# tsurumeso/vocal-remover

Measured on NVIDIA H100. Metric: seconds-of-audio/sec separated (n_fft=2048, hop=1024), higher is better.
Workload: dtype bf16x3 (split-bf16 operands hi+lo, 3 wgmma passes, fp32 accumulate); fft/lstm fp32

## Files before the change

### vocal-remover_b200/build.py

```python
import os
import subprocess
import sys
from concurrent.futures import ThreadPoolExecutor

HERE = os.path.dirname(os.path.abspath(__file__))
CSRC = os.path.join(HERE, 'csrc')
OBJ = os.path.join(HERE, 'build')
LIB = os.path.join(HERE, 'libvr_b200.so')
SOURCES = ['api.cu', 'engine.cu', 'conv_simt.cu', 'conv_tc.cu', 'conv_tc_rows.cu', 'conv_tc_halo.cu', 'elementwise.cu', 'lstm.cu', 'fft.cu', 'resample.cu', 'flac.cu', 'flac_encode.cu']
NVCC = os.environ.get('NVCC', '/usr/local/cuda/bin/nvcc')
FLAGS = ['-gencode', 'arch=compute_90a,code=sm_90a', '-O3', '-lineinfo', '-std=c++17',
         '-Xcompiler', '-fPIC', '-Xcompiler', '-fvisibility=hidden', '--expt-relaxed-constexpr']


def _newest_header():
    hs = [os.path.join(CSRC, f) for f in os.listdir(CSRC) if f.endswith(('.h', '.cuh'))]
    hs.append(os.path.join(HERE, '..', 'include', 'vr_b200.h'))
    return max(os.path.getmtime(h) for h in hs)


def build(verbose=False, force=False):
    global OBJ, LIB
    extra = os.environ.get('VR_BUILD_FLAGS', '').split()
    if os.environ.get('VR_BUILD_TAG'):
        OBJ = os.path.join(HERE, 'build_' + os.environ['VR_BUILD_TAG'])
        LIB = os.path.join(HERE, 'libvr_b200_%s.so' % os.environ['VR_BUILD_TAG'])
    os.makedirs(OBJ, exist_ok=True)
    hdr = _newest_header()
    jobs = []
    for src in SOURCES:
        s = os.path.join(CSRC, src)
        o = os.path.join(OBJ, src.replace('.cu', '.o'))
        if force or not os.path.exists(o) or os.path.getmtime(o) < max(os.path.getmtime(s), hdr):
            jobs.append((s, o))

    def cc(job):
        s, o = job
        cmd = [NVCC] + FLAGS + extra + ['-c', s, '-o', o]
        if verbose:
            cmd += ['-Xptxas', '-v']
        r = subprocess.run(cmd, capture_output=True, text=True)
        if r.returncode != 0:
            raise RuntimeError('nvcc failed for %s:\n%s\n%s' % (s, r.stdout, r.stderr))
        return r.stderr

    with ThreadPoolExecutor(max_workers=min(8, max(1, len(jobs)))) as ex:
        logs = list(ex.map(cc, jobs))
    if verbose:
        for lg in logs:
            print(lg)
    objs = [os.path.join(OBJ, s.replace('.cu', '.o')) for s in SOURCES]
    if jobs or not os.path.exists(LIB):
        cmd = [NVCC, '-shared', '-o', LIB] + objs + ['-gencode', 'arch=compute_90a,code=sm_90a']
        r = subprocess.run(cmd, capture_output=True, text=True)
        if r.returncode != 0:
            raise RuntimeError('link failed:\n%s\n%s' % (r.stdout, r.stderr))
    return LIB


if __name__ == '__main__':
    print(build(verbose='-v' in sys.argv, force='-f' in sys.argv))
```

### vocal-remover_b200/csrc/api.cu

```cuda
#include <stdio.h>
#include <string.h>

#include <string>

#include "../../include/vr_b200.h"
#include "engine.h"
#include "kernels.h"
#include "tc_plan.h"

struct vr_ctx {
  vr::Engine* eng;
  std::string err;
};

static std::string g_create_err;

static int fail(vr_ctx* c, const std::string& m) {
  if (c) c->err = m;
  return -1;
}
static int done(vr_ctx* c, bool ok) {
  if (ok) return 0;
  c->err = c->eng->err;
  return -1;
// ... 255 lines not shown
  cudaError_t e = cudaMalloc(&p, (size_t)bytes);
  if (e != cudaSuccess) return fail(ctx, std::string("vr_shared_alloc: cudaMalloc: ") + cudaGetErrorString(e));
  cudaIpcMemHandle_t h;
  e = cudaIpcGetMemHandle(&h, p);
  if (e != cudaSuccess) {
    cudaFree(p);
    return fail(ctx, std::string("vr_shared_alloc: cudaIpcGetMemHandle: ") + cudaGetErrorString(e));
  }
  memcpy(handle64, &h, 64);
  *dev_ptr = p;
  return 0;
}

int vr_shared_open(vr_ctx* ctx, const unsigned char* handle64, void** dev_ptr) {
  CHECK_CTX(ctx);
  if (!dev_ptr || !handle64) return fail(ctx, "vr_shared_open: bad arguments");
  cudaIpcMemHandle_t h;
  memcpy(&h, handle64, 64);
  void* p = nullptr;
  cudaError_t e = cudaIpcOpenMemHandle(&p, h, cudaIpcMemLazyEnablePeerAccess);
  if (e != cudaSuccess) return fail(ctx, std::string("vr_shared_open: cudaIpcOpenMemHandle: ") + cudaGetErrorString(e));
  *dev_ptr = p;
  return 0;
}

int vr_shared_close(vr_ctx* ctx, void* dev_ptr, int32_t owner) {
  CHECK_CTX(ctx);
  if (!dev_ptr) return 0;
  cudaError_t e = owner ? cudaFree(dev_ptr) : cudaIpcCloseMemHandle(dev_ptr);
  if (e != cudaSuccess) return fail(ctx, std::string("vr_shared_close: ") + cudaGetErrorString(e));
  return 0;
}

int64_t vr_launch_count(const vr_ctx* ctx) { return ctx && ctx->eng ? ctx->eng->launches : 0; }

int vr_profile_enable(vr_ctx* ctx, int32_t on) {
  CHECK_CTX(ctx);
  ctx->eng->profile_enable(on != 0);
  return 0;
}

int vr_profile_read(vr_ctx* ctx, double* out6) {
  CHECK_CTX(ctx);
  return done(ctx, ctx->eng->profile_read(out6));
}

int vr_profile_dump(vr_ctx* ctx, char* text, int64_t cap, int64_t* needed) {
  CHECK_CTX(ctx);
  std::string t;
  if (!ctx->eng->profile_dump(t)) return done(ctx, false);
  if (needed) *needed = (int64_t)t.size() + 1;
  if (text && cap > 0) {
    const size_t n = t.size() < (size_t)cap - 1 ? t.size() : (size_t)cap - 1;
    memcpy(text, t.data(), n);
    text[n] = 0;
  }
  return 0;
}

int vr_debug_conv(vr_ctx* ctx, const float* x, int32_t N, int32_t Cin, int32_t H, int32_t W, const float* w,
                  const float* bias, int32_t Cout, int32_t k, int32_t stride, int32_t dil_h, int32_t dil_w, int32_t act,
                  int32_t use_tc, float* y, void* stream) {
  CHECK_CTX(ctx);
  return done(ctx, ctx->eng->debug_conv(x, N, Cin, H, W, w, bias, Cout, k, stride, dil_h, dil_w, act, use_tc, y,
                                        (cudaStream_t)stream));
}

int vr_debug_decoder(vr_ctx* ctx, const float* low, int32_t N, int32_t Cl, int32_t h, int32_t w, const float* skip,
                     int32_t Cs, const float* wgt, const float* bias, int32_t Cout, int32_t act, int32_t fused, float* y,
                     void* stream) {
  CHECK_CTX(ctx);
  return done(ctx, ctx->eng->debug_decoder(low, N, Cl, h, w, skip, Cs, wgt, bias, Cout, act, fused, y,
                                           (cudaStream_t)stream));
}

int vr_debug_tensor(vr_ctx* ctx, const char* name, int32_t n0, int32_t n, float* out, int64_t* shape4, void* stream) {
  CHECK_NET(ctx);
  if (!name || !shape4) return fail(ctx, "vr_debug_tensor: name and shape4 are required");
  return done(ctx, ctx->eng->debug_tensor(name, n0, n, out, shape4, (cudaStream_t)stream));
}

int vr_debug_set(int32_t key, int32_t value) {
  int* knob = key == 0 ? &vr::g_debug.trace : key == 2 ? &vr::g_debug.rows_wide : key == 3 ? &vr::g_debug.halo
            : key == 6 ? &vr::g_debug.kskip : key == 7 ? &vr::g_debug.crop_mask : nullptr;
  if (!knob) return -1;
  *knob = value;
  return 0;
}

int64_t vr_debug_trace(uint64_t* host_out, int64_t capacity) {
  return vr::tc_rows_read_trace((unsigned long long*)host_out, (long long)capacity);
}

}
```

### vocal-remover_b200/csrc/conv_tc.cu

```cuda
#include <cuda.h>
#include <stdio.h>

#include <map>
#include <tuple>

#include "engine.h"
#include "tc_common.cuh"
#include "tc_plan.h"

namespace vr {

static constexpr int kMaxStages = 8;
static constexpr int kConsumerWarps = 8;
static constexpr int kThreads = 32 * kConsumerWarps + 32;
static constexpr int kStaticSmem = 2048;

struct TcParams {
  int N, Ho, Wo, Wt, Ht, Nt, tiles_w, tiles_h, m_tiles, n_tiles;
  int stride, pad_h, pad_w, dil_h, dil_w, KW;
  int cchunks, total_sub, CinPadTC, Cout, act, stages;
  bf16* out_hi;
  bf16* out_lo;
  int64_t osn, osh;
  int osw;
// ... 73 lines not shown
    __syncwarp();
  } else {
    const int wg = warp >> 2;
    const float slope = act_slope(p.act);
    const uint32_t dhi = desc_hi(8 * KB * 2, kLayout);
    MbarRing ring(smem_u32(&bar_full[0]), smem_u32(&bar_empty[0]), 0, p.stages);
    float acc[BN / 2];
    for (int tile = blockIdx.x; tile < total_tiles; tile += gridDim.x) {
#pragma unroll
      for (int i = 0; i < BN / 2; ++i) acc[i] = 0.f;
      HeldSlot held;
      for (int it = 0; it < num_iters; ++it) {
        const int nsub = min(SUBS, p.total_sub - it * SUBS);
        ring.wait_full();
        const uint32_t sdesc = desc_lo(smem_base + (uint32_t)ring.slot * kStageBytes);
        wg_fence();
#pragma unroll
        for (int j = 0; j < SUBS; ++j) {
          if (j < nsub) {
            const uint32_t a_hi = sdesc + ((j * kASub + (uint32_t)wg * (kAPlane / 2)) >> 4);
            const uint32_t a_lo = a_hi + (kAPlane >> 4);
            const uint32_t b_hi = sdesc + ((kBRegion + j * kBSub) >> 4);
            const uint32_t b_lo = b_hi + (kBPlane >> 4);
#pragma unroll
            for (int k = 0; k < kSteps; ++k)
              wgmma_split3<BN>(acc, a_hi + 2u * k, a_lo + 2u * k, b_hi + 2u * k, b_lo + 2u * k, dhi);
          }
        }
        wg_commit();
        wg_wait<1>();
        held.release(ring, lane);
        held.hold(ring);
        ring.advance();
      }
      wg_wait<0>();
      held.release_last(ring, lane);

      const int nt = tile % p.n_tiles;
      const int mt = tile / p.n_tiles;
      const int w0 = (mt % p.tiles_w) * p.Wt;
      const int h0 = ((mt / p.tiles_w) % p.tiles_h) * p.Ht;
      const int n0 = (mt / (p.tiles_w * p.tiles_h)) * p.Nt;
      const int c_lane = nt * BN + 2 * (lane & 3);
#pragma unroll
      for (int hr = 0; hr < 2; ++hr) {
        const int row = 64 * wg + 16 * (warp & 3) + (lane >> 2) + 8 * hr;
        const int dw = row % p.Wt;
        const int dh = (row / p.Wt) % p.Ht;
        const int n = n0 + row / (p.Wt * p.Ht);
        if (n >= p.N) continue;
        const int64_t obase = (int64_t)n * p.osn + (int64_t)(h0 + dh) * p.osh + (int64_t)(w0 + dw) * p.osw;
#pragma unroll
        for (int j = 0; j < BN / 8; ++j)
          epilogue_pair(acc[4 * j + 2 * hr], acc[4 * j + 2 * hr + 1], bias_s, c_lane + 8 * j, p.Cout, slope,
                        p.out_hi + obase, p.out_lo + obase);
      }
    }
  }
}

#define VR_TC_FOR_BN(X, KB) X(KB, 16) X(KB, 32) X(KB, 48) X(KB, 64) X(KB, 80) X(KB, 96) X(KB, 112) X(KB, 128)
#define VR_TC_FOR_ALL(X) VR_TC_FOR_BN(X, 64) VR_TC_FOR_BN(X, 32) VR_TC_FOR_BN(X, 16)


TcDebug g_debug;

static constexpr int kMaxDevices = 64;
const TcDevice& tc_device() {
  static TcDevice table[kMaxDevices];
  static TcDevice none;
  int dev = -1;
  if (cudaGetDevice(&dev) != cudaSuccess || dev < 0 || dev >= kMaxDevices) return none;
  TcDevice& d = table[dev];
  if (!d.ok) {
    if (cudaDeviceGetAttribute(&d.max_smem, cudaDevAttrMaxSharedMemoryPerBlockOptin, dev) != cudaSuccess ||
        cudaDeviceGetAttribute(&d.num_sms, cudaDevAttrMultiProcessorCount, dev) != cudaSuccess)
      return none;
#define VR_TC_SET_SMEM(KB, BN) \
  cudaFuncSetAttribute(conv_tc_kernel<KB, BN>, cudaFuncAttributeMaxDynamicSharedMemorySize, d.max_smem - kStaticSmem);
    VR_TC_FOR_ALL(VR_TC_SET_SMEM)
#undef VR_TC_SET_SMEM
    tc_rows_set_attributes(d.max_smem);
    tc_halo_set_attributes(d.max_smem);
    d.ok = true;
  }
  return d;
}

typedef CUresult (*EncodeTiledFn)(CUtensorMap*, CUtensorMapDataType, cuuint32_t, void*, const cuuint64_t*,
                                  const cuuint64_t*, const cuuint32_t*, const cuuint32_t*, CUtensorMapInterleave,
                                  CUtensorMapSwizzle, CUtensorMapL2promotion, CUtensorMapFloatOOBfill);
static EncodeTiledFn tc_encode_fn() {
  static EncodeTiledFn fn = nullptr;
  if (!fn) {
    void* p = nullptr;
    cudaDriverEntryPointQueryResult q;
    if (cudaGetDriverEntryPoint("cuTensorMapEncodeTiled", &p, cudaEnableDefault, &q) == cudaSuccess &&
        q == cudaDriverEntryPointSuccess)
      fn = (EncodeTiledFn)p;
  }
  return fn;
}

static CUtensorMapSwizzle swizzle_for(int KB) {
  return KB == 64 ? CU_TENSOR_MAP_SWIZZLE_128B : KB == 32 ? CU_TENSOR_MAP_SWIZZLE_64B : CU_TENSOR_MAP_SWIZZLE_32B;
}

static uint16_t tc_f2bf(float f) {
  uint32_t u;
  memcpy(&u, &f, 4);
  if ((u & 0x7fffffffu) > 0x7f800000u) return (uint16_t)((u >> 16) | 0x40);
  uint32_t r = 0x7fffu + ((u >> 16) & 1u);
  return (uint16_t)((u + r) >> 16);
}
static float tc_bf2f(uint16_t h) {
  uint32_t u = (uint32_t)h << 16;
  float f;
  memcpy(&f, &u, 4);
  return f;
}

struct TileGeom {
  int Wt, Ht, Nt;
  bool ok;
};
static TileGeom tile_geom(int Ho, int Wo) {
  TileGeom g{0, 0, 0, false};
  if (Wo <= 0 || Ho <= 0) return g;
  if (Wo >= 128) {
    if (Wo % 128) return g;
    g.Wt = 128; g.Ht = 1; g.Nt = 1;
  } else {
    if (128 % Wo) return g;
    g.Wt = Wo;
    g.Ht = 128 / Wo < Ho ? 128 / Wo : Ho;
    if (Ho % g.Ht) return g;
    if ((128 / Wo) % g.Ht) return g;
    g.Nt = 128 / (g.Wt * g.Ht);
  }
  g.ok = true;
  return g;
}

struct NTiling {
  int BN, n_tiles;
};
static NTiling n_tiling(const ConvLayer& L, bool rows, bool rows_wide) {
  const int cout16 = round_up(L.Cout, 16);
  if (rows) {
    const int BN = cout16 == 16 ? 16 : (rows_wide && cout16 % 64 == 0 ? 64 : 32);
    return {BN, ceil_div(cout16, BN)};
  }
  const int n_tiles = ceil_div(cout16, 128);
  return {round_up(ceil_div(cout16, n_tiles), 16), n_tiles};
}

TcKind tc_choose(const ConvLayer& L, int H, int W, bool rows_wide) {
  if (!(L.k == 1 || L.k == 3) || !(L.stride == 1 || L.stride == 2) || L.Cout < 4) return TC_NONE;
  const TileGeom g = tile_geom(H, W);
  if (!g.ok || g.Wt * L.stride > 256 || g.Ht * L.stride > 256) return TC_NONE;
  const bool k3s1 = L.k == 3 && L.stride == 1 && L.dil_h == 1 && L.dil_w == 1;
  const NTiling r = n_tiling(L, true, rows_wide), t = n_tiling(L, false, false);
  if (k3s1 && W % 128 == 0 && H % 8 == 0 && tc_rows_has(r.BN) && r.n_tiles * r.BN <= 256) return TC_ROWS;
  if (k3s1 && (W == 16 || W == 32 || W == 64) && H % (128 / W) == 0 && tc_halo_has(t.BN) &&
      t.n_tiles * t.BN <= 256 && g_debug.halo != 1)
    return TC_HALO;
  if (t.n_tiles * t.BN > 256) return TC_NONE;
  return TC_GENERIC;
}

template <class At>
static std::vector<uint16_t> split_bf16(const ConvLayer& L, const float* wp, int rows, int K, At at) {
  std::vector<uint16_t> planes((size_t)2 * rows * K, 0);
  const size_t lo = (size_t)rows * K;
  for (int co = 0; co < L.Cout; ++co)
    for (int t = 0; t < L.k * L.k; ++t)
      for (int ci = 0; ci < L.CinPad; ++ci) {
        const float w = wp[((size_t)t * L.CinPad + ci) * L.CoutPad + co];
        const uint16_t hi = tc_f2bf(w);
        const size_t i = at(co, t, ci);
        planes[i] = hi;
        planes[lo + i] = tc_f2bf(w - tc_bf2f(hi));
      }
  return planes;
}

static unsigned long long weight_group_mask(const ConvLayer& L, const float* wp, int CinPad) {
  if (CinPad / 8 > 64) return ~0ull;
  unsigned long long m = 0x3ull;
  for (int ci = 0; ci < L.CinPad; ++ci) {
    bool any = false;
    for (int t = 0; t < L.k * L.k && !any; ++t)
      for (int co = 0; co < L.Cout && !any; ++co) any = wp[((size_t)t * L.CinPad + ci) * L.CoutPad + co] != 0.f;
    if (any) m |= 1ull << (ci / 8);
  }
  return m;
}

static bool encode_weight_map(TcConv& tc, int rows, int K, int box_rows, std::string& err, const std::string& name) {
  cuuint64_t dims[3] = {(cuuint64_t)K, (cuuint64_t)rows, 2};
  cuuint64_t strides[2] = {(cuuint64_t)K * 2, (cuuint64_t)rows * K * 2};
  cuuint32_t box[3] = {(cuuint32_t)tc.KB, (cuuint32_t)box_rows, 2};
  cuuint32_t es[3] = {1, 1, 1};
  CUresult r = tc_encode_fn()(&tc.map_b, CU_TENSOR_MAP_DATA_TYPE_BFLOAT16, 3, tc.w_planes.get(), dims, strides, box, es,
                              CU_TENSOR_MAP_INTERLEAVE_NONE, swizzle_for(tc.KB), CU_TENSOR_MAP_L2_PROMOTION_L2_256B,
                              CU_TENSOR_MAP_FLOAT_OOB_FILL_NONE);
  if (r != CUDA_SUCCESS) {
    err = "cuTensorMapEncodeTiled(weights) failed for " + name + " code " + std::to_string((int)r);
    return false;
  }
  return true;
}

const CUtensorMap* tc_activation_map(TcConv& tc, const ActView& v, int bw, int bh, int bn, int es, std::string& err,
                                     const std::string& name) {
  const ViewKey key = std::make_tuple((const void*)v.hi, (const void*)v.lo, v.N, v.H, v.W, v.C, bw, bh, bn);
  auto it = tc.map_a.find(key);
  if (it != tc.map_a.end()) return &it->second;
  const int64_t plane = (const char*)v.lo - (const char*)v.hi;
  if (v.sw % 8 || v.sh % 8 || v.sn % 8 || (reinterpret_cast<uintptr_t>(v.hi) & 15) || plane <= 0 || plane % 16) {
    err = "internal: the input of " + name + " is not 16-byte aligned or its lo plane does not follow its hi plane";
    return nullptr;
  }
  cuuint64_t dims[5] = {(cuuint64_t)v.C, (cuuint64_t)v.W, (cuuint64_t)v.H, (cuuint64_t)v.N, 2};
  cuuint64_t strides[4] = {(cuuint64_t)v.sw * 2, (cuuint64_t)v.sh * 2, (cuuint64_t)v.sn * 2, (cuuint64_t)plane};
  cuuint32_t box[5] = {(cuuint32_t)tc.KB, (cuuint32_t)bw, (cuuint32_t)bh, (cuuint32_t)bn, 2};
  cuuint32_t estr[5] = {1, (cuuint32_t)es, (cuuint32_t)es, 1, 1};
  CUtensorMap m;
  CUresult r = tc_encode_fn()(&m, CU_TENSOR_MAP_DATA_TYPE_BFLOAT16, 5, (void*)v.hi, dims, strides, box, estr,
                              CU_TENSOR_MAP_INTERLEAVE_NONE, swizzle_for(tc.KB), CU_TENSOR_MAP_L2_PROMOTION_L2_256B,
                              CU_TENSOR_MAP_FLOAT_OOB_FILL_NONE);
  if (r != CUDA_SUCCESS) {
    err = "cuTensorMapEncodeTiled(activations) failed for " + name + " code " + std::to_string((int)r);
    return nullptr;
  }
  return &tc.map_a.emplace(key, m).first->second;
}

bool tc_prepare(ConvLayer& L, const float* w, const float* b, int H, int W, bool rows_wide, std::string& err) {
  const TcKind kind = tc_choose(L, H, W, rows_wide);
  if (kind == TC_NONE) return true;
  if (!tc_encode_fn()) {
    err = "cuTensorMapEncodeTiled is not available from the driver";
    return false;
  }
  auto tc = std::make_shared<TcConv>();
  tc->kind = kind;
  tc->H = H; tc->W = W;
  const NTiling nt = n_tiling(L, kind == TC_ROWS, rows_wide);
  const int BN = nt.BN, cin16 = round_up(L.CinPad, 16);
  tc->BN = BN; tc->n_tiles = nt.n_tiles;
  tc->KB = kind != TC_GENERIC ? 32 : cin16 % 64 == 0 ? 64 : cin16 % 32 == 0 ? 32 : 16;
  const int CinPad = round_up(L.CinPad, tc->KB);
  tc->CinPad = CinPad;
  tc->chunks = CinPad / tc->KB;
  tc->kmask = weight_group_mask(L, w, CinPad);
  const int rows = nt.n_tiles * BN;
  std::vector<uint16_t> planes;
  int brows, K;
  if (kind == TC_ROWS) {
    brows = 3 * rows;
    K = 3 * CinPad;
    planes = split_bf16(L, w, brows, K, [&](int co, int t, int ci) {
      return (size_t)(co / BN * 3 * BN + (2 - t / 3) * BN + co % BN) * K + (size_t)(t % 3) * CinPad + ci;
    });
  } else {
    brows = rows;
    K = L.k * L.k * CinPad;
    planes = split_bf16(L, w, brows, K, [&](int co, int t, int ci) { return (size_t)co * K + (size_t)t * CinPad + ci; });
  }
  std::vector<float> bias((size_t)rows, 0.f);
  for (int co = 0; co < L.Cout; ++co) bias[(size_t)co] = b[co];
  if (tc->w_planes.alloc(planes.size() * 2) != cudaSuccess || tc->bias.alloc(bias.size() * 4) != cudaSuccess) {
    err = "cudaMalloc failed while packing tensor-core weights for " + L.name;
    return false;
  }
  if (!upload(tc->w_planes.get(), planes.data(), planes.size() * 2, err) ||
      !upload(tc->bias.get(), bias.data(), bias.size() * 4, err) ||
      !encode_weight_map(*tc, brows, K, kind == TC_ROWS ? 3 * BN : BN, err, L.name))
    return false;
  L.tc = tc;
  return true;
}

cudaError_t tc_launch(const ConvLayer& L, const ActView& in, const ActView& out, cudaStream_t s, std::string& err,
                      const ConvFusion& f) {
  TcConv& tc = *L.tc;
  if (out.H != tc.H || out.W != tc.W || (in.H - 1) / L.stride + 1 != out.H || (in.W - 1) / L.stride + 1 != out.W) {
    err = "internal: " + L.name + " is launched on maps of another size than it was prepared for";
    return cudaErrorInvalidValue;
  }
  if (tc.kind == TC_ROWS) return tc_rows_launch(L, tc, in, out, s, err, f);
  if (!f.empty()) {
    err = "tc_launch: fused work is only implemented in the row-streaming kernel";
    return cudaErrorInvalidValue;
  }
  if (tc.kind == TC_HALO) return tc_halo_launch(L, tc, in, out, s, err);
  const TileGeom g = tile_geom(out.H, out.W);
  const CUtensorMap* map_a = tc_activation_map(tc, in, g.Wt * L.stride, g.Ht * L.stride, g.Nt, L.stride, err, L.name);
  if (!map_a) return cudaErrorInvalidValue;
  const int SUBS = 64 / tc.KB;
  TcParams p;
  p.N = out.N; p.Ho = out.H; p.Wo = out.W;
  p.Wt = g.Wt; p.Ht = g.Ht; p.Nt = g.Nt;
  p.tiles_w = out.W / g.Wt; p.tiles_h = out.H / g.Ht;
  p.m_tiles = p.tiles_w * p.tiles_h * ceil_div(out.N, g.Nt);
  p.n_tiles = tc.n_tiles;
  p.stride = L.stride; p.dil_h = L.dil_h; p.dil_w = L.dil_w;
  p.pad_h = L.dil_h * (L.k / 2); p.pad_w = L.dil_w * (L.k / 2);
  p.KW = L.k;
  p.cchunks = tc.chunks; p.total_sub = L.k * L.k * tc.chunks;
  p.CinPadTC = tc.CinPad; p.Cout = L.Cout; p.act = L.act;
  const int stage_bytes = SUBS * (2 * 128 * tc.KB * 2 + 2 * tc.BN * tc.KB * 2);
  const TcDevice& dv = tc_device();
  if (!dv.ok) {
    err = "tc_launch: cannot query the current device";
    return cudaErrorInvalidValue;
  }
  const int dyn = dv.max_smem - kStaticSmem;
  p.stages = (dyn - 1024) / stage_bytes;
  if (p.stages > kMaxStages) p.stages = kMaxStages;
  if (p.stages < 2) {
    err = "tc_launch: shared memory too small for two pipeline stages";
    return cudaErrorInvalidValue;
  }
  p.out_hi = out.hi; p.out_lo = out.lo;
  p.osn = out.sn; p.osh = out.sh; p.osw = out.sw;
  p.bias = tc.bias.get();
  const int total_tiles = p.m_tiles * p.n_tiles;
  const int grid = total_tiles < dv.num_sms ? total_tiles : dv.num_sms;
#define VR_TC_LAUNCH(KB_, BN_)                                                       \
  if (tc.KB == KB_ && tc.BN == BN_) {                                                \
    conv_tc_kernel<KB_, BN_><<<grid, kThreads, dyn, s>>>(*map_a, tc.map_b, p);       \
    return cudaGetLastError();                                                       \
  }
  VR_TC_FOR_ALL(VR_TC_LAUNCH)
#undef VR_TC_LAUNCH
  err = "tc_launch: no kernel instantiation for this channel tile";
  return cudaErrorInvalidValue;
}

}
```

### vocal-remover_b200/csrc/tc_common.cuh

```cuda
#pragma once
#include <cuda.h>
#include <stdint.h>
#include <stdio.h>

#include "common.cuh"

namespace vr {

__device__ __forceinline__ uint32_t smem_u32(const void* p) { return (uint32_t)__cvta_generic_to_shared(p); }

__device__ __forceinline__ bool elect_one_sync() {
  uint32_t pred;
  asm volatile(
      "{\n\t"
      ".reg .pred P1;\n\t"
      "elect.sync _|P1, 0xffffffff;\n\t"
      "selp.u32 %0, 1, 0, P1;\n\t"
      "}"
      : "=r"(pred));
  return pred != 0;
}

__device__ __forceinline__ void mbar_init(uint32_t bar, uint32_t count) {
  asm volatile("mbarrier.init.shared::cta.b64 [%0], %1;" ::"r"(bar), "r"(count));
// ... 21 lines not shown
      "WAIT_DONE:\n\t"
      "}" ::"r"(bar),
      "r"(parity)
      : "memory");
#else
  asm volatile(
      "{\n\t"
      ".reg .pred p;\n\t"
      "WAIT_LOOP:\n\t"
      "mbarrier.try_wait.parity.shared::cta.b64 p, [%0], %1;\n\t"
      "@p bra WAIT_DONE;\n\t"
      "bra WAIT_LOOP;\n\t"
      "WAIT_DONE:\n\t"
      "}" ::"r"(bar),
      "r"(parity)
      : "memory");
#endif
}
__device__ __forceinline__ void warp_arrive(uint32_t bar, int lane) {
  __syncwarp();
  if (lane == 0) mbar_arrive(bar);
}

struct MbarRing {
  uint32_t full0, empty0;
  int lo, hi, slot;
  uint32_t phase;

  __device__ __forceinline__ MbarRing(uint32_t full0_, uint32_t empty0_, int lo_, int hi_)
      : full0(full0_), empty0(empty0_), lo(lo_), hi(hi_), slot(lo_), phase(0) {}
  __device__ __forceinline__ uint32_t full(int s) const { return full0 + (uint32_t)s * 8u; }
  __device__ __forceinline__ uint32_t empty(int s) const { return empty0 + (uint32_t)s * 8u; }
  __device__ __forceinline__ uint32_t full() const { return full(slot); }
  __device__ __forceinline__ uint32_t empty() const { return empty(slot); }
  __device__ __forceinline__ void wait_full() const { mbar_wait(full(), phase); }
  __device__ __forceinline__ void wait_empty() const { mbar_wait(empty(), phase ^ 1u); }
  __device__ __forceinline__ void advance() {
    if (++slot == hi) {
      slot = lo;
      phase ^= 1u;
    }
  }
  __device__ __forceinline__ void init(uint32_t full_count, uint32_t empty_count) const {
    for (int s = lo; s < hi; ++s) {
      mbar_init(full(s), full_count);
      mbar_init(empty(s), empty_count);
    }
  }
};

struct HeldSlot {
  int slot = -1;
  __device__ __forceinline__ void hold(const MbarRing& r) { slot = r.slot; }
  __device__ __forceinline__ void release(const MbarRing& r, int lane) {
    if (slot >= 0) {
      warp_arrive(r.empty(slot), lane);
      slot = -1;
    }
  }
  __device__ __forceinline__ void release_last(const MbarRing& r, int lane) {
    warp_arrive(r.empty(slot), lane);
    slot = -1;
  }
};

__device__ __forceinline__ void tma_prefetch(const CUtensorMap* map) {
  asm volatile("prefetch.tensormap [%0];" ::"l"(map) : "memory");
}
__device__ __forceinline__ void tma_load_5d(uint32_t dst, const CUtensorMap* map, int c0, int c1, int c2, int c3,
                                            int c4, uint32_t bar) {
  asm volatile(
      "cp.async.bulk.tensor.5d.shared::cluster.global.tile.mbarrier::complete_tx::bytes [%0], [%1, {%2, %3, %4, %5, "
      "%6}], [%7];" ::"r"(dst),
      "l"(map), "r"(c0), "r"(c1), "r"(c2), "r"(c3), "r"(c4), "r"(bar)
      : "memory");
}
__device__ __forceinline__ void tma_load_3d(uint32_t dst, const CUtensorMap* map, int c0, int c1, int c2,
                                            uint32_t bar) {
  asm volatile(
      "cp.async.bulk.tensor.3d.shared::cluster.global.tile.mbarrier::complete_tx::bytes [%0], [%1, {%2, %3, %4}], "
      "[%5];" ::"r"(dst),
      "l"(map), "r"(c0), "r"(c1), "r"(c2), "r"(bar)
      : "memory");
}

__device__ __forceinline__ uint32_t desc_lo(uint32_t addr) { return ((addr & 0x3FFFFu) >> 4) | (1u << 16); }
__device__ __forceinline__ uint32_t desc_hi(uint32_t sbo_bytes, uint32_t layout_type) {
  return (sbo_bytes >> 4) | (layout_type << 30);
}
__device__ __forceinline__ uint64_t desc64(uint32_t lo, uint32_t hi) { return ((uint64_t)hi << 32) | lo; }

__device__ __forceinline__ void wg_fence() { asm volatile("wgmma.fence.sync.aligned;" ::: "memory"); }
__device__ __forceinline__ void wg_commit() { asm volatile("wgmma.commit_group.sync.aligned;" ::: "memory"); }
template <int PENDING>
__device__ __forceinline__ void wg_wait() {
  asm volatile("wgmma.wait_group.sync.aligned %0;" ::"n"(PENDING) : "memory");
}

template <int N>
struct Wgmma;
template <>
struct Wgmma<16> {
  static __device__ __forceinline__ void mma(float* d, uint64_t a, uint64_t b) {
    asm volatile(
        "wgmma.mma_async.sync.aligned.m64n16k16.f32.bf16.bf16 {%0, %1, %2, %3, %4, %5, %6, %7}, %8, %9, 1, 1, 1, 0, 0;"
        : "+f"(d[0]), "+f"(d[1]), "+f"(d[2]), "+f"(d[3]), "+f"(d[4]), "+f"(d[5]), "+f"(d[6]), "+f"(d[7])
        : "l"(a), "l"(b)
        : "memory");
  }
};
template <>
struct Wgmma<32> {
  static __device__ __forceinline__ void mma(float* d, uint64_t a, uint64_t b) {
    asm volatile(
        "wgmma.mma_async.sync.aligned.m64n32k16.f32.bf16.bf16 {%0, %1, %2, %3, %4, %5, %6, %7, %8, %9, %10, %11, %12, %13, %14, %15}, %16, %17, 1, 1, 1, 0, 0;"
        : "+f"(d[0]), "+f"(d[1]), "+f"(d[2]), "+f"(d[3]), "+f"(d[4]), "+f"(d[5]), "+f"(d[6]), "+f"(d[7]), "+f"(d[8]), "+f"(d[9]), "+f"(d[10]), "+f"(d[11]), "+f"(d[12]), "+f"(d[13]), "+f"(d[14]), "+f"(d[15])
        : "l"(a), "l"(b)
        : "memory");
  }
};
template <>
struct Wgmma<48> {
  static __device__ __forceinline__ void mma(float* d, uint64_t a, uint64_t b) {
    asm volatile(
        "wgmma.mma_async.sync.aligned.m64n48k16.f32.bf16.bf16 {%0, %1, %2, %3, %4, %5, %6, %7, %8, %9, %10, %11, %12, %13, %14, %15, %16, %17, %18, %19, %20, %21, %22, %23}, %24, %25, 1, 1, 1, 0, 0;"
        : "+f"(d[0]), "+f"(d[1]), "+f"(d[2]), "+f"(d[3]), "+f"(d[4]), "+f"(d[5]), "+f"(d[6]), "+f"(d[7]), "+f"(d[8]), "+f"(d[9]), "+f"(d[10]), "+f"(d[11]), "+f"(d[12]), "+f"(d[13]), "+f"(d[14]), "+f"(d[15]), "+f"(d[16]), "+f"(d[17]), "+f"(d[18]), "+f"(d[19]), "+f"(d[20]), "+f"(d[21]), "+f"(d[22]), "+f"(d[23])
        : "l"(a), "l"(b)
        : "memory");
  }
};
template <>
struct Wgmma<64> {
  static __device__ __forceinline__ void mma(float* d, uint64_t a, uint64_t b) {
    asm volatile(
        "wgmma.mma_async.sync.aligned.m64n64k16.f32.bf16.bf16 {%0, %1, %2, %3, %4, %5, %6, %7, %8, %9, %10, %11, %12, %13, %14, %15, %16, %17, %18, %19, %20, %21, %22, %23, %24, %25, %26, %27, %28, %29, %30, %31}, %32, %33, 1, 1, 1, 0, 0;"
        : "+f"(d[0]), "+f"(d[1]), "+f"(d[2]), "+f"(d[3]), "+f"(d[4]), "+f"(d[5]), "+f"(d[6]), "+f"(d[7]), "+f"(d[8]), "+f"(d[9]), "+f"(d[10]), "+f"(d[11]), "+f"(d[12]), "+f"(d[13]), "+f"(d[14]), "+f"(d[15]), "+f"(d[16]), "+f"(d[17]), "+f"(d[18]), "+f"(d[19]), "+f"(d[20]), "+f"(d[21]), "+f"(d[22]), "+f"(d[23]), "+f"(d[24]), "+f"(d[25]), "+f"(d[26]), "+f"(d[27]), "+f"(d[28]), "+f"(d[29]), "+f"(d[30]), "+f"(d[31])
        : "l"(a), "l"(b)
        : "memory");
  }
};
template <>
struct Wgmma<80> {
  static __device__ __forceinline__ void mma(float* d, uint64_t a, uint64_t b) {
    asm volatile(
        "wgmma.mma_async.sync.aligned.m64n80k16.f32.bf16.bf16 {%0, %1, %2, %3, %4, %5, %6, %7, %8, %9, %10, %11, %12, %13, %14, %15, %16, %17, %18, %19, %20, %21, %22, %23, %24, %25, %26, %27, %28, %29, %30, %31, %32, %33, %34, %35, %36, %37, %38, %39}, %40, %41, 1, 1, 1, 0, 0;"
        : "+f"(d[0]), "+f"(d[1]), "+f"(d[2]), "+f"(d[3]), "+f"(d[4]), "+f"(d[5]), "+f"(d[6]), "+f"(d[7]), "+f"(d[8]), "+f"(d[9]), "+f"(d[10]), "+f"(d[11]), "+f"(d[12]), "+f"(d[13]), "+f"(d[14]), "+f"(d[15]), "+f"(d[16]), "+f"(d[17]), "+f"(d[18]), "+f"(d[19]), "+f"(d[20]), "+f"(d[21]), "+f"(d[22]), "+f"(d[23]), "+f"(d[24]), "+f"(d[25]), "+f"(d[26]), "+f"(d[27]), "+f"(d[28]), "+f"(d[29]), "+f"(d[30]), "+f"(d[31]), "+f"(d[32]), "+f"(d[33]), "+f"(d[34]), "+f"(d[35]), "+f"(d[36]), "+f"(d[37]), "+f"(d[38]), "+f"(d[39])
        : "l"(a), "l"(b)
        : "memory");
  }
};
template <>
struct Wgmma<96> {
  static __device__ __forceinline__ void mma(float* d, uint64_t a, uint64_t b) {
    asm volatile(
        "wgmma.mma_async.sync.aligned.m64n96k16.f32.bf16.bf16 {%0, %1, %2, %3, %4, %5, %6, %7, %8, %9, %10, %11, %12, %13, %14, %15, %16, %17, %18, %19, %20, %21, %22, %23, %24, %25, %26, %27, %28, %29, %30, %31, %32, %33, %34, %35, %36, %37, %38, %39, %40, %41, %42, %43, %44, %45, %46, %47}, %48, %49, 1, 1, 1, 0, 0;"
        : "+f"(d[0]), "+f"(d[1]), "+f"(d[2]), "+f"(d[3]), "+f"(d[4]), "+f"(d[5]), "+f"(d[6]), "+f"(d[7]), "+f"(d[8]), "+f"(d[9]), "+f"(d[10]), "+f"(d[11]), "+f"(d[12]), "+f"(d[13]), "+f"(d[14]), "+f"(d[15]), "+f"(d[16]), "+f"(d[17]), "+f"(d[18]), "+f"(d[19]), "+f"(d[20]), "+f"(d[21]), "+f"(d[22]), "+f"(d[23]), "+f"(d[24]), "+f"(d[25]), "+f"(d[26]), "+f"(d[27]), "+f"(d[28]), "+f"(d[29]), "+f"(d[30]), "+f"(d[31]), "+f"(d[32]), "+f"(d[33]), "+f"(d[34]), "+f"(d[35]), "+f"(d[36]), "+f"(d[37]), "+f"(d[38]), "+f"(d[39]), "+f"(d[40]), "+f"(d[41]), "+f"(d[42]), "+f"(d[43]), "+f"(d[44]), "+f"(d[45]), "+f"(d[46]), "+f"(d[47])
        : "l"(a), "l"(b)
        : "memory");
  }
};
template <>
struct Wgmma<112> {
  static __device__ __forceinline__ void mma(float* d, uint64_t a, uint64_t b) {
    asm volatile(
        "wgmma.mma_async.sync.aligned.m64n112k16.f32.bf16.bf16 {%0, %1, %2, %3, %4, %5, %6, %7, %8, %9, %10, %11, %12, %13, %14, %15, %16, %17, %18, %19, %20, %21, %22, %23, %24, %25, %26, %27, %28, %29, %30, %31, %32, %33, %34, %35, %36, %37, %38, %39, %40, %41, %42, %43, %44, %45, %46, %47, %48, %49, %50, %51, %52, %53, %54, %55}, %56, %57, 1, 1, 1, 0, 0;"
        : "+f"(d[0]), "+f"(d[1]), "+f"(d[2]), "+f"(d[3]), "+f"(d[4]), "+f"(d[5]), "+f"(d[6]), "+f"(d[7]), "+f"(d[8]), "+f"(d[9]), "+f"(d[10]), "+f"(d[11]), "+f"(d[12]), "+f"(d[13]), "+f"(d[14]), "+f"(d[15]), "+f"(d[16]), "+f"(d[17]), "+f"(d[18]), "+f"(d[19]), "+f"(d[20]), "+f"(d[21]), "+f"(d[22]), "+f"(d[23]), "+f"(d[24]), "+f"(d[25]), "+f"(d[26]), "+f"(d[27]), "+f"(d[28]), "+f"(d[29]), "+f"(d[30]), "+f"(d[31]), "+f"(d[32]), "+f"(d[33]), "+f"(d[34]), "+f"(d[35]), "+f"(d[36]), "+f"(d[37]), "+f"(d[38]), "+f"(d[39]), "+f"(d[40]), "+f"(d[41]), "+f"(d[42]), "+f"(d[43]), "+f"(d[44]), "+f"(d[45]), "+f"(d[46]), "+f"(d[47]), "+f"(d[48]), "+f"(d[49]), "+f"(d[50]), "+f"(d[51]), "+f"(d[52]), "+f"(d[53]), "+f"(d[54]), "+f"(d[55])
// ... 145 lines not shown
```

### vocal-remover_b200/csrc/tc_plan.h

```cpp
#pragma once
#include <cuda.h>

#include <map>
#include <tuple>

#include "engine.h"

namespace vr {

enum TcKind {
  TC_NONE,
  TC_GENERIC,
  TC_ROWS,
  TC_HALO,
};

typedef std::tuple<const void*, const void*, int, int, int, int, int, int, int> ViewKey;

struct TcConv {
  TcKind kind = TC_NONE;
  int H = 0, W = 0;
  int KB = 0, CinPad = 0, chunks = 0, BN = 0, n_tiles = 0;
  unsigned long long kmask = ~0ull;
  DevPtr<bf16> w_planes;
  DevPtr<float> bias;
  CUtensorMap map_b;
  std::map<ViewKey, CUtensorMap> map_a;
  bool fuses_upsample(int up_C) const { return kind == TC_ROWS && up_C % 32 == 0 && up_C <= CinPad; }
  bool fuses_dot() const { return kind == TC_ROWS; }
  bool fuses_mask(int Cout, int offset, bool up) const {
    const int kept = W - 2 * offset;
    return kind == TC_ROWS && up && n_tiles == 1 && BN <= 32 && BN == Cout && offset >= 0 && kept > 0 &&
           kept % 128 == 0;
  }
};

TcKind tc_choose(const ConvLayer& L, int H, int W, bool rows_wide);
const CUtensorMap* tc_activation_map(TcConv& tc, const ActView& v, int bw, int bh, int bn, int es, std::string& err,
                                     const std::string& name);

cudaError_t tc_rows_launch(const ConvLayer& L, TcConv& tc, const ActView& in, const ActView& out, cudaStream_t s,
                           std::string& err, const ConvFusion& f);
void tc_rows_set_attributes(int max_smem);
bool tc_rows_has(int BN);
int tc_rows_read_trace(unsigned long long* out, long long capacity);

cudaError_t tc_halo_launch(const ConvLayer& L, TcConv& tc, const ActView& in, const ActView& out, cudaStream_t s,
                           std::string& err);
void tc_halo_set_attributes(int max_smem);
bool tc_halo_has(int BN);

struct TcDevice {
  bool ok = false;
  int num_sms = 0, max_smem = 0;
};
const TcDevice& tc_device();

struct TcDebug {
  int trace = 0;
  int rows_wide = 0;
  int halo = 0;
  int kskip = 1;
  int crop_mask = 1;
};
extern TcDebug g_debug;

}
```

Baseline: 2810.

## Add dedicated stride-2 3x3 tensor-core conv kernel with polyphase window reuse

Adds a new warp-specialized kernel for 3x3 stride-2 convolutions. It loads four polyphase (even/odd row/column) sub-windows of the input once per channel chunk via TMA and reuses them across all nine taps through ldmatrix register fragments. Weights are streamed with bulk copies into a deep ring, and the kernel is persistent with register reallocation between producer and consumer warps. It is selected for shallow-channel encoder layers in place of the generic kernel, which reloads a strided tile per tap. The cost is more code paths and added shared-memory pressure.

```diff
diff --git a/vocal-remover_b200/build.py b/vocal-remover_b200/build.py
--- a/vocal-remover_b200/build.py
+++ b/vocal-remover_b200/build.py
@@ -7,7 +7,7 @@
 CSRC = os.path.join(HERE, 'csrc')
 OBJ = os.path.join(HERE, 'build')
 LIB = os.path.join(HERE, 'libvr_b200.so')
-SOURCES = ['api.cu', 'engine.cu', 'conv_simt.cu', 'conv_tc.cu', 'conv_tc_rows.cu', 'conv_tc_halo.cu', 'elementwise.cu', 'lstm.cu', 'fft.cu', 'resample.cu', 'flac.cu', 'flac_encode.cu']
+SOURCES = ['api.cu', 'engine.cu', 'conv_simt.cu', 'conv_tc.cu', 'conv_tc_rows.cu', 'conv_tc_halo.cu', 'conv_tc_s2.cu', 'elementwise.cu', 'lstm.cu', 'fft.cu', 'resample.cu', 'flac.cu', 'flac_encode.cu']
 NVCC = os.environ.get('NVCC', '/usr/local/cuda/bin/nvcc')
 FLAGS = ['-gencode', 'arch=compute_90a,code=sm_90a', '-O3', '-lineinfo', '-std=c++17',
          '-Xcompiler', '-fPIC', '-Xcompiler', '-fvisibility=hidden', '--expt-relaxed-constexpr']
diff --git a/vocal-remover_b200/csrc/api.cu b/vocal-remover_b200/csrc/api.cu
--- a/vocal-remover_b200/csrc/api.cu
+++ b/vocal-remover_b200/csrc/api.cu
@@ -361,7 +361,8 @@
 
 int vr_debug_set(int32_t key, int32_t value) {
   int* knob = key == 0 ? &vr::g_debug.trace : key == 2 ? &vr::g_debug.rows_wide : key == 3 ? &vr::g_debug.halo
-            : key == 6 ? &vr::g_debug.kskip : key == 7 ? &vr::g_debug.crop_mask : nullptr;
+            : key == 6 ? &vr::g_debug.kskip : key == 7 ? &vr::g_debug.crop_mask
+            : key == 8 ? &vr::g_debug.s2 : nullptr;
   if (!knob) return -1;
   *knob = value;
   return 0;
diff --git a/vocal-remover_b200/csrc/conv_tc.cu b/vocal-remover_b200/csrc/conv_tc.cu
--- a/vocal-remover_b200/csrc/conv_tc.cu
+++ b/vocal-remover_b200/csrc/conv_tc.cu
@@ -179,6 +179,7 @@
 #undef VR_TC_SET_SMEM
     tc_rows_set_attributes(d.max_smem);
     tc_halo_set_attributes(d.max_smem);
+    tc_s2_set_attributes(d.max_smem);
     d.ok = true;
   }
   return d;
@@ -263,6 +264,10 @@
       t.n_tiles * t.BN <= 256 && g_debug.halo != 1)
     return TC_HALO;
   if (t.n_tiles * t.BN > 256) return TC_NONE;
+  const bool s2_tiles = L.k == 3 && L.stride == 2 && L.dil_h == 1 && L.dil_w == 1 &&
+                        (W == 16 || W == 32 || W == 64 || W == 128) && H % tc_s2_tile_rows(W) == 0 && tc_s2_has(t.BN);
+  const int cin16 = round_up(L.CinPad, 16);
+  if (s2_tiles && g_debug.s2 != 1 && (cin16 == 16 || (cin16 == 32 && W == 128) || g_debug.s2 == 2)) return TC_S2;
   return TC_GENERIC;
 }
 
@@ -347,7 +352,7 @@
   const NTiling nt = n_tiling(L, kind == TC_ROWS, rows_wide);
   const int BN = nt.BN, cin16 = round_up(L.CinPad, 16);
   tc->BN = BN; tc->n_tiles = nt.n_tiles;
-  tc->KB = kind != TC_GENERIC ? 32 : cin16 % 64 == 0 ? 64 : cin16 % 32 == 0 ? 32 : 16;
+  tc->KB = kind == TC_S2 ? 16 : kind != TC_GENERIC ? 32 : cin16 % 64 == 0 ? 64 : cin16 % 32 == 0 ? 32 : 16;
   const int CinPad = round_up(L.CinPad, tc->KB);
   tc->CinPad = CinPad;
   tc->chunks = CinPad / tc->KB;
@@ -361,6 +366,15 @@
     planes = split_bf16(L, w, brows, K, [&](int co, int t, int ci) {
       return (size_t)(co / BN * 3 * BN + (2 - t / 3) * BN + co % BN) * K + (size_t)(t % 3) * CinPad + ci;
     });
+  } else if (kind == TC_S2) {
+    brows = rows;
+    K = 9 * CinPad;
+    const int hchunks = CinPad / 16;
+    planes = split_bf16(L, w, brows, K, [&](int co, int t, int ci) {
+      const int r = co % BN, c = ci % 16;
+      return ((size_t)((co / BN) * 9 + t) * hchunks + ci / 16) * BN * 16 + (size_t)r * 16 +
+             (size_t)(((c >> 3) ^ ((r >> 2) & 1)) << 3) + (c & 7);
+    });
   } else {
     brows = rows;
     K = L.k * L.k * CinPad;
@@ -374,7 +388,7 @@
   }
   if (!upload(tc->w_planes.get(), planes.data(), planes.size() * 2, err) ||
       !upload(tc->bias.get(), bias.data(), bias.size() * 4, err) ||
-      !encode_weight_map(*tc, brows, K, kind == TC_ROWS ? 3 * BN : BN, err, L.name))
+      (kind != TC_S2 && !encode_weight_map(*tc, brows, K, kind == TC_ROWS ? 3 * BN : BN, err, L.name)))
     return false;
   L.tc = tc;
   return true;
@@ -393,6 +407,7 @@
     return cudaErrorInvalidValue;
   }
   if (tc.kind == TC_HALO) return tc_halo_launch(L, tc, in, out, s, err);
+  if (tc.kind == TC_S2) return tc_s2_launch(L, tc, in, out, s, err);
   const TileGeom g = tile_geom(out.H, out.W);
   const CUtensorMap* map_a = tc_activation_map(tc, in, g.Wt * L.stride, g.Ht * L.stride, g.Nt, L.stride, err, L.name);
   if (!map_a) return cudaErrorInvalidValue;
diff --git a/vocal-remover_b200/csrc/conv_tc_s2.cu b/vocal-remover_b200/csrc/conv_tc_s2.cu
--- /dev/null
+++ b/vocal-remover_b200/csrc/conv_tc_s2.cu
@@ -0,0 +1,300 @@
+#include <stdio.h>
+
+#include "engine.h"
+#include "tc_common.cuh"
+#include "tc_plan.h"
+
+namespace vr {
+
+static constexpr int kConsumerWarps = 8;
+static constexpr int kProducerWarps = 4;
+static constexpr int kThreads = 32 * (kConsumerWarps + kProducerWarps);
+static constexpr int kLaunchRegs = 168;
+static constexpr int kConsumerRegs = 232;
+static constexpr int kProducerRegs = 40;
+static_assert(kConsumerWarps * kConsumerRegs + kProducerWarps * kProducerRegs <=
+                  (kConsumerWarps + kProducerWarps) * kLaunchRegs,
+              "setmaxnreg.inc would wait forever for registers the block does not own");
+static constexpr int kStaticSmem = 2048;
+static constexpr int kMaxASlots = 4;
+static constexpr int kMaxWStages = 18;
+static constexpr uint32_t kKB = 16;
+static constexpr uint32_t kRowB = kKB * 2;
+static constexpr int kTilePx = 256;
+
+template <int BN>
+struct S2Geom {
+  static constexpr uint32_t kBPlane = BN * kRowB;
+  static constexpr uint32_t kWStage = 2 * kBPlane;
+};
+
+struct S2Maps {
+  CUtensorMap a[4];
+};
+
+struct S2Params {
+  int lw, Wt, Ht, tiles_w, tiles_h, n_tiles, total_tiles;
+  int hchunks, CinPad, Cout, act;
+  int n_aslots, n_wstages;
+  uint32_t aslot;
+  uint32_t sub_off[4];
+  uint32_t sub_plane[4];
+  const bf16* w;
+  int64_t w_plane;
+  unsigned long long kmask;
+  bf16* out_hi;
+  bf16* out_lo;
+  int64_t osn, osh;
+  int osw;
+  const float* bias;
+};
+
+__device__ __forceinline__ uint32_t half_chunk_groups(unsigned long long kmask, int hc) {
+  const int sh = hc * 2;
+  return sh + 2 <= 64 ? (uint32_t)(kmask >> sh) & 0x3u : 0x3u;
+}
+
+struct S2Consumer {
+  MbarRing a, w;
+  HeldSlot held_w;
+};
+
+template <int BN>
+__device__ __forceinline__ void consume_s2(S2Consumer& st, const S2Params& p, float* acc, uint32_t (&fr)[3][16],
+                                           const uint32_t* qe, const uint32_t* qo, uint32_t a_base, uint32_t w_base,
+                                           uint32_t dhi, int lane) {
+  typedef S2Geom<BN> G;
+  st.a.wait_full();
+  const uint32_t slot = a_base + (uint32_t)st.a.slot * p.aslot;
+#pragma unroll
+  for (int t = 0; t < 9; ++t) {
+    const int kh = t / 3, kw = t % 3;
+    const int s = 2 * (kh & 1) + (kw & 1);
+    uint32_t* f = fr[t % 3];
+#pragma unroll
+    for (int b = 0; b < 2; ++b) {
+      const uint32_t q = (kw & 1) ? qo[b] + (uint32_t)((kh >> 1) * p.Wt)
+                                  : qe[b] + (uint32_t)((kh >> 1) * (p.Wt + 8) + (kw >> 1));
+      const uint32_t a = slot + p.sub_off[s] + (q << 5) + ((((uint32_t)lane >> 4) ^ ((q >> 2) & 1u)) << 4);
+      ldsm_x4(f + 8 * b, a);
+      ldsm_x4(f + 8 * b + 4, a + p.sub_plane[s]);
+    }
+    st.w.wait_full();
+    const uint32_t b_hi = desc_lo(w_base + (uint32_t)st.w.slot * G::kWStage);
+    wg_fence();
+#pragma unroll
+    for (int b = 0; b < 2; ++b)
+      wgmma_split3_rs<BN>(acc + b * (BN / 2), f + 8 * b, f + 8 * b + 4, b_hi, b_hi + (G::kBPlane >> 4), dhi);
+    wg_commit();
+    if (t == 8) warp_arrive(st.a.empty(), lane);
+    wg_wait<1>();
+    st.held_w.release(st.w, lane);
+    st.held_w.hold(st.w);
+    st.w.advance();
+  }
+  st.a.advance();
+}
+
+template <int BN>
+__global__ void __launch_bounds__(kThreads, 1)
+    conv_s2_kernel(const __grid_constant__ S2Maps tmA, const S2Params p) {
+  typedef S2Geom<BN> G;
+  extern __shared__ uint8_t smem_raw[];
+  __shared__ __align__(8) uint64_t bar_afull[kMaxASlots];
+  __shared__ __align__(8) uint64_t bar_aempty[kMaxASlots];
+  __shared__ __align__(8) uint64_t bar_wfull[kMaxWStages];
+  __shared__ __align__(8) uint64_t bar_wempty[kMaxWStages];
+  __shared__ float bias_s[256];
+
+  const int warp = __shfl_sync(0xffffffffu, (int)threadIdx.x >> 5, 0);
+  const int lane = threadIdx.x & 31;
+  const uint32_t smem_base = (smem_u32(smem_raw) + 1023u) & ~1023u;
+  const uint32_t a_base = smem_base;
+  const uint32_t w_base = smem_base + (uint32_t)p.n_aslots * p.aslot;
+  MbarRing aring(smem_u32(&bar_afull[0]), smem_u32(&bar_aempty[0]), 0, p.n_aslots);
+  MbarRing wring(smem_u32(&bar_wfull[0]), smem_u32(&bar_wempty[0]), 0, p.n_wstages);
+
+  if (warp == kConsumerWarps && lane == 0) {
+#pragma unroll
+    for (int s = 0; s < 4; ++s) tma_prefetch(&tmA.a[s]);
+    aring.init(1, kConsumerWarps);
+    wring.init(1, kConsumerWarps);
+    asm volatile("fence.mbarrier_init.release.cluster;" ::: "memory");
+  }
+  for (int i = threadIdx.x; i < p.n_tiles * BN; i += blockDim.x) bias_s[i] = __ldg(p.bias + i);
+  __syncthreads();
+
+  if (warp >= kConsumerWarps) {
+    setmaxnreg_dec<kProducerRegs>();
+    if (warp == kConsumerWarps && elect_one_sync()) {
+      for (int tile = blockIdx.x; tile < p.total_tiles; tile += gridDim.x) {
+        const int mt = tile / p.n_tiles;
+        const int w0 = (mt % p.tiles_w) * p.Wt;
+        const int h0 = ((mt / p.tiles_w) % p.tiles_h) * p.Ht;
+        const int n = mt / (p.tiles_w * p.tiles_h);
+#pragma unroll 1
+        for (int hc = 0; hc < p.hchunks; ++hc) {
+          if (!half_chunk_groups(p.kmask, hc)) continue;
+          aring.wait_empty();
+          mbar_expect_tx(aring.full(), p.aslot);
+          const uint32_t slot = a_base + (uint32_t)aring.slot * p.aslot;
+#pragma unroll
+          for (int s = 0; s < 4; ++s)
+            tma_load_5d(slot + p.sub_off[s], &tmA.a[s], hc * (int)kKB, 2 * w0 - 1 + (s & 1), 2 * h0 - 1 + (s >> 1), n,
+                        0, aring.full());
+          aring.advance();
+        }
+      }
+    } else if (warp == kConsumerWarps + 1 && elect_one_sync()) {
+      const uint32_t tap_elems = (uint32_t)p.hchunks * (BN * kKB);
+      for (int tile = blockIdx.x; tile < p.total_tiles; tile += gridDim.x) {
+        const bf16* nt_w = p.w + (size_t)(tile % p.n_tiles) * 9 * tap_elems;
+#pragma unroll 1
+        for (int hc = 0; hc < p.hchunks; ++hc) {
+          if (!half_chunk_groups(p.kmask, hc)) continue;
+          const bf16* src = nt_w + (size_t)hc * (BN * kKB);
+#pragma unroll 1
+          for (int t = 0; t < 9; ++t, src += tap_elems) {
+            wring.wait_empty();
+            mbar_expect_tx(wring.full(), G::kWStage);
+            const uint32_t dst = w_base + (uint32_t)wring.slot * G::kWStage;
+            bulk_load(dst, src, G::kBPlane, wring.full());
+            bulk_load(dst + G::kBPlane, src + p.w_plane, G::kBPlane, wring.full());
+            wring.advance();
+          }
+        }
+      }
+    }
+    __syncwarp();
+  } else {
+    setmaxnreg_inc<kConsumerRegs>();
+    const int wg = warp >> 2;
+    const float slope = act_slope(p.act);
+    const uint32_t dhi = desc_hi(8 * kRowB, 3u);
+    uint32_t qe[2], qo[2];
+#pragma unroll
+    for (int b = 0; b < 2; ++b) {
+      const int px = 64 * (2 * wg + b) + 16 * (warp & 3) + (lane & 15);
+      const int i = px >> p.lw, j = px & (p.Wt - 1);
+      qe[b] = (uint32_t)(i * (p.Wt + 8) + j);
+      qo[b] = (uint32_t)(i * p.Wt + j);
+    }
+    S2Consumer st{aring, wring};
+    float acc[BN];
+    uint32_t fr[3][16];
+    for (int tile = blockIdx.x; tile < p.total_tiles; tile += gridDim.x) {
+#pragma unroll
+      for (int i = 0; i < BN; ++i) acc[i] = 0.f;
+      for (int hc = 0; hc < p.hchunks; ++hc) {
+        if (!half_chunk_groups(p.kmask, hc)) continue;
+        consume_s2<BN>(st, p, acc, fr, qe, qo, a_base, w_base, dhi, lane);
+      }
+      wg_wait<0>();
+      st.held_w.release_last(st.w, lane);
+
+      const int nt = tile % p.n_tiles;
+      const int mt = tile / p.n_tiles;
+      const int w0 = (mt % p.tiles_w) * p.Wt;
+      const int h0 = ((mt / p.tiles_w) % p.tiles_h) * p.Ht;
+      const int n = mt / (p.tiles_w * p.tiles_h);
+      const int c_lane = nt * BN + 2 * (lane & 3);
+#pragma unroll
+      for (int b = 0; b < 2; ++b) {
+#pragma unroll
+        for (int hr = 0; hr < 2; ++hr) {
+          const int px = 64 * (2 * wg + b) + 16 * (warp & 3) + (lane >> 2) + 8 * hr;
+          const int64_t obase = (int64_t)n * p.osn + (int64_t)(h0 + (px >> p.lw)) * p.osh +
+                                (int64_t)(w0 + (px & (p.Wt - 1))) * p.osw;
+          const float* v = acc + b * (BN / 2) + 2 * hr;
+#pragma unroll
+          for (int j = 0; j < BN / 8; ++j)
+            epilogue_pair(v[4 * j], v[4 * j + 1], bias_s, c_lane + 8 * j, p.Cout, slope, p.out_hi + obase,
+                          p.out_lo + obase);
+        }
+      }
+    }
+  }
+}
+
+#define VR_S2_FOR_ALL(X) X(16) X(32) X(48) X(64) X(96) X(128)
+
+bool tc_s2_has(int BN) {
+#define VR_S2_HAS(BN_) if (BN == BN_) return true;
+  VR_S2_FOR_ALL(VR_S2_HAS)
+#undef VR_S2_HAS
+  return false;
+}
+
+int tc_s2_tile_rows(int W) { return kTilePx / (W < 64 ? W : 64); }
+
+cudaError_t tc_s2_launch(const ConvLayer& L, TcConv& tc, const ActView& in, const ActView& out, cudaStream_t s,
+                         std::string& err) {
+  const TcDevice& dv = tc_device();
+  if (!dv.ok) {
+    err = "tc_s2_launch: cannot query the current device";
+    return cudaErrorInvalidValue;
+  }
+  S2Params p;
+  p.Wt = out.W < 64 ? out.W : 64;
+  p.lw = p.Wt == 16 ? 4 : p.Wt == 32 ? 5 : 6;
+  p.Ht = kTilePx / p.Wt;
+  if (out.H % p.Ht || out.W % p.Wt) {
+    err = "internal: " + L.name + " does not tile into the stride-2 kernel's 256-pixel tiles";
+    return cudaErrorInvalidValue;
+  }
+  p.tiles_w = out.W / p.Wt;
+  p.tiles_h = out.H / p.Ht;
+  p.n_tiles = tc.n_tiles;
+  p.total_tiles = out.N * p.tiles_h * p.tiles_w * p.n_tiles;
+  p.hchunks = tc.chunks; p.CinPad = tc.CinPad; p.Cout = L.Cout; p.act = L.act;
+  p.kmask = g_debug.kskip == 1 ? tc.kmask : ~0ull;
+  p.w = tc.w_planes.get();
+  p.w_plane = (int64_t)tc.n_tiles * tc.BN * 9 * tc.CinPad;
+  p.out_hi = out.hi; p.out_lo = out.lo;
+  p.osn = out.sn; p.osh = out.sh; p.osw = out.sw;
+  p.bias = tc.bias.get();
+  S2Maps maps;
+  uint32_t off = 0;
+  for (int sb = 0; sb < 4; ++sb) {
+    const int rows = (sb >> 1) ? p.Ht : p.Ht + 1;
+    const int cols = (sb & 1) ? p.Wt : p.Wt + 8;
+    const CUtensorMap* m = tc_activation_map(tc, in, 2 * cols, 2 * rows, 1, 2, err, L.name);
+    if (!m) return cudaErrorInvalidValue;
+    maps.a[sb] = *m;
+    p.sub_off[sb] = off;
+    p.sub_plane[sb] = (uint32_t)(rows * cols) * kRowB;
+    off += 2 * p.sub_plane[sb];
+  }
+  p.aslot = off;
+  const int w_stage = tc.BN * 2 * (int)kRowB;
+  const int dyn = dv.max_smem - kStaticSmem;
+  const int avail = dyn - 1024;
+  p.n_aslots = (avail - 9 * w_stage) / (int)p.aslot;
+  if (p.n_aslots > kMaxASlots) p.n_aslots = kMaxASlots;
+  if (p.n_aslots < 2) p.n_aslots = 2;
+  p.n_wstages = (avail - p.n_aslots * (int)p.aslot) / w_stage;
+  if (p.n_wstages > kMaxWStages) p.n_wstages = kMaxWStages;
+  if (p.n_wstages < 2) {
+    err = "tc_s2_launch: shared memory too small for two window slots and two weight stages";
+    return cudaErrorInvalidValue;
+  }
+  const int grid = p.total_tiles < dv.num_sms ? p.total_tiles : dv.num_sms;
+#define VR_S2_LAUNCH(BN_)                                                \
+  if (tc.BN == BN_) {                                                    \
+    conv_s2_kernel<BN_><<<grid, kThreads, dyn, s>>>(maps, p);            \
+    return cudaGetLastError();                                           \
+  }
+  VR_S2_FOR_ALL(VR_S2_LAUNCH)
+#undef VR_S2_LAUNCH
+  err = "tc_s2_launch: no kernel instantiation for this channel tile";
+  return cudaErrorInvalidValue;
+}
+
+void tc_s2_set_attributes(int max_smem) {
+#define VR_S2_SET(BN_) \
+  cudaFuncSetAttribute(conv_s2_kernel<BN_>, cudaFuncAttributeMaxDynamicSharedMemorySize, max_smem - kStaticSmem);
+  VR_S2_FOR_ALL(VR_S2_SET)
+#undef VR_S2_SET
+}
+
+}
diff --git a/vocal-remover_b200/csrc/tc_common.cuh b/vocal-remover_b200/csrc/tc_common.cuh
--- a/vocal-remover_b200/csrc/tc_common.cuh
+++ b/vocal-remover_b200/csrc/tc_common.cuh
@@ -127,6 +127,12 @@
       "[%5];" ::"r"(dst),
       "l"(map), "r"(c0), "r"(c1), "r"(c2), "r"(bar)
       : "memory");
+}
+
+__device__ __forceinline__ void bulk_load(uint32_t dst, const void* src, uint32_t bytes, uint32_t bar) {
+  asm volatile("cp.async.bulk.shared::cluster.global.mbarrier::complete_tx::bytes [%0], [%1], %2, [%3];" ::"r"(dst),
+               "l"(src), "r"(bytes), "r"(bar)
+               : "memory");
 }
 
 __device__ __forceinline__ uint32_t desc_lo(uint32_t addr) { return ((addr & 0x3FFFFu) >> 4) | (1u << 16); }
diff --git a/vocal-remover_b200/csrc/tc_plan.h b/vocal-remover_b200/csrc/tc_plan.h
--- a/vocal-remover_b200/csrc/tc_plan.h
+++ b/vocal-remover_b200/csrc/tc_plan.h
@@ -13,6 +13,7 @@
   TC_GENERIC,
   TC_ROWS,
   TC_HALO,
+  TC_S2,
 };
 
 typedef std::tuple<const void*, const void*, int, int, int, int, int, int, int> ViewKey;
@@ -50,6 +51,12 @@
 void tc_halo_set_attributes(int max_smem);
 bool tc_halo_has(int BN);
 
+cudaError_t tc_s2_launch(const ConvLayer& L, TcConv& tc, const ActView& in, const ActView& out, cudaStream_t s,
+                         std::string& err);
+void tc_s2_set_attributes(int max_smem);
+bool tc_s2_has(int BN);
+int tc_s2_tile_rows(int W);
+
 struct TcDevice {
   bool ok = false;
   int num_sms = 0, max_smem = 0;
@@ -62,6 +69,7 @@
   int halo = 0;
   int kskip = 1;
   int crop_mask = 1;
+  int s2 = 0;
 };
 extern TcDebug g_debug;
 
```

Result: faster. 2851 (median of 6 runs) (+1.5%).
